# worldbench/lidarcrafter

Hardware: AMD Instinct MI355X
Metric: denoising-steps/sec, nuScenes 32×1024 range image, 1/2/4/8 GPU (higher is better)
Workload: dtype f16x2-split MFMA, fp32 accumulate (fp32-class accuracy)

## Files before the change

lidarcrafter_amd/csrc/conv_f16x2_s2.hip:

```cpp
#include "conv_f16x2_common.h"

using namespace lcconv;

namespace {

#include "conv_f16x2_ps.h"

typedef _Float16 half8_s2 __attribute__((ext_vector_type(8)));

__global__ __launch_bounds__(256) void fir_down2_prefilter_split_kernel(
    const float* __restrict__ x, long long x_bs, half8_s2* __restrict__ ysp, int C8, int H, int W, int nstrip, int strip_len,
    lc_conv_range* range) {
    const int Wh = W >> 1;
    const int i = blockIdx.x * 256 + threadIdx.x;
    const int c8 = blockIdx.y;
    const int b = blockIdx.z / nstrip, strip = blockIdx.z - b * nstrip;
    const float xs = range->x_scale, seen = range->amax_scaled;
    float am = 0.f;
    if (i < Wh) {
        const long long HW = (long long)H * W;
        const float* xb = x + b * x_bs + (long long)c8 * 8 * HW;
        const int R = H + 3;
        half8_s2* yh = ysp + ((long long)b * 2 * C8 + c8) * R * W;
        half8_s2* yl = yh + (long long)C8 * R * W;
        const int cm1 = (2 * i - 1 + W) % W, cp2 = (2 * i + 2) % W;
        constexpr float f0 = 0.125f, f1 = 0.375f, f2 = 0.375f, f3 = 0.125f;
        struct Raw { float a[8]; float2 m[8], c[8]; };
        auto load_raw = [&](int r, Raw& w) {
            const int rc = r < 0 ? 0 : (r >= H ? H - 1 : r);
            const float* p = xb + (long long)rc * W;
#pragma unroll
            for (int k = 0; k < 8; ++k) {
                const float* q = p + (long long)k * HW;
                w.a[k] = q[cm1];
                w.m[k] = *reinterpret_cast<const float2*>(q + 2 * i);
                w.c[k] = *reinterpret_cast<const float2*>(q + cp2);
            }
        };
        auto xw_row = [&](int r, const Raw& w, float (&e)[8], float (&o)[8]) {
            const float in = (r >= 0 && r < H) ? 1.0f : 0.0f;
#pragma unroll
            for (int k = 0; k < 8; ++k) {
                e[k] = in * fmaf(f3, w.c[k].x, fmaf(f2, w.m[k].y, fmaf(f1, w.m[k].x, f0 * w.a[k])));
                o[k] = in * fmaf(f3, w.c[k].y, fmaf(f2, w.c[k].x, fmaf(f1, w.m[k].y, f0 * w.m[k].x)));
            }
        };
        auto put = [&](int row, const float (&e)[8], const float (&o)[8]) {
            half8 h, l;
            split8(e, xs, h, l, am);
            yh[(long long)row * W + Wh + i] = h;
            yl[(long long)row * W + Wh + i] = l;
            const int jo = i + 1 == Wh ? 0 : i + 1;
            split8(o, xs, h, l, am);
            yh[(long long)row * W + jo] = h;
            yl[(long long)row * W + jo] = l;
        };
        const int m0 = -1 + strip * strip_len;
        const int m1 = (m0 + strip_len < H) ? m0 + strip_len : H;
        float we[4][8], wo[4][8];
        Raw raw;
        load_raw(m0 - 1, raw); xw_row(m0 - 1, raw, we[0], wo[0]);
        load_raw(m0, raw); xw_row(m0, raw, we[1], wo[1]);
        load_raw(m0 + 1, raw); xw_row(m0 + 1, raw, we[2], wo[2]);
        load_raw(m0 + 2, raw);
        for (int m = m0; m < m1; ++m) {
            xw_row(m + 2, raw, we[3], wo[3]);
            if (m + 1 < m1) load_raw(m + 3, raw);
            float fe[8], fo[8];
#pragma unroll
            for (int k = 0; k < 8; ++k) {
                fe[k] = fmaf(f3, we[3][k], fmaf(f2, we[2][k], fmaf(f1, we[1][k], f0 * we[0][k])));
                fo[k] = fmaf(f3, wo[3][k], fmaf(f2, wo[2][k], fmaf(f1, wo[1][k], f0 * wo[0][k])));
            }
            put(m + 1, fe, fo);
            if (m == 1) {
#pragma unroll
                for (int k = 0; k < 8; ++k) {
                    fe[k] = fmaf(f3, we[3][k], fmaf(f2, we[2][k], f1 * we[1][k]));
                    fo[k] = fmaf(f3, wo[3][k], fmaf(f2, wo[2][k], f1 * wo[1][k]));
                }
                put(H + 1, fe, fo);
            }
            if (m == H - 3) {
#pragma unroll
                for (int k = 0; k < 8; ++k) {
                    fe[k] = fmaf(f2, we[2][k], fmaf(f1, we[1][k], f0 * we[0][k]));
                    fo[k] = fmaf(f2, wo[2][k], fmaf(f1, wo[1][k], f0 * wo[0][k]));
                }
                put(H + 2, fe, fo);
            }
#pragma unroll
            for (int k = 0; k < 8; ++k) {
                we[0][k] = we[1][k]; we[1][k] = we[2][k]; we[2][k] = we[3][k];
                wo[0][k] = wo[1][k]; wo[1][k] = wo[2][k]; wo[2][k] = wo[3][k];
            }
        }
    }
    publish_amax(range, am, seen);
}

using S2Cfg_ = HCfg<2, 2, 1, 1, 1, 64, 3>;

template <int TPB, bool EMIT_STATS>
__global__ __launch_bounds__(256, 1) void conv_s2_shared_w_kernel(ConvArgsH a) {
    using C = S2Cfg_;
    constexpr int CB = 2, NTAP = 9, BN = 64, TW = 64;
    constexpr int XW = 2 * TW + 1, XR = 3, XU = CB * XR * XW, WU = NTAP * CB * BN;
    constexpr int NWV = 4;
    constexpr int NXI = (XU + 63) / 64, NWI = (WU + 63) / 64;
    constexpr int XS = NXI * 64, WS = NWI * 64;
    constexpr int KX = (2 * NXI + NWV - 1) / NWV, KW = (2 * NWI + NWV - 1) / NWV;
    constexpr unsigned OOB = 0x80000000u;
    __shared__ half8 xlds[2][2 * XS];
    __shared__ half8 wlds[2][2 * WS];
    __shared__ half8 dummy[64];
    const int tid = threadIdx.x, lane = tid & 63;
    const int wave = __builtin_amdgcn_readfirstlane(tid >> 6);
    const int wco = wave >> 1, wpx = wave & 1;
    const int kh = lane >> 5, l31 = lane & 31;

    int bx = blockIdx.x;
    if (a.xcd) bx = (bx & 7) * (gridDim.x >> 3) + (bx >> 3);
    const int gh_ = a.tiles_h / TPB;
    const int tw_i = bx % a.tiles_w; bx /= a.tiles_w;
    const int h0 = (bx % gh_) * TPB; bx /= gh_;
    const int b = bx;
    const int w0 = tw_i * TW;
    const int co0 = blockIdx.y * BN;
    const int H = a.H, W = a.W, HW = H * W;
// ... 176 lines not shown
            for (int m = 0; m < 4; ++m) {
                const int co_oct = co0 + wco * 32 + 8 * m;
                const float sh = half_sum_to_lane31_63(st_s[m]), qh = half_sum_to_lane31_63(st_q[m]);
                const float sf = dpp_add<0x143, 0xC>(sh), qf = dpp_add<0x143, 0xC>(qh);
                const int ent = quads ? (co_oct >> 2) + (lane >> 5) : (co_oct >> 3);
                const unsigned eo = (mine && co_oct < a.Co && gh < H)
                                        ? ((unsigned)ent * (unsigned)a.oslots + (unsigned)slot) * 16u + 4u * (lane & 3)
                                        : OOB;
                store_entry_4lanes(rs_o, st_p[m], nv, quads ? sh : sf, quads ? qh : qf, eo);
            }
        }
    }
}

using S2Cfg = HCfg<2, 2, 1, 1, 1, 64, 3>;

}

extern "C" int64_t lc_conv2d_ring_s2_stats_slots(int Ho, int Wo) {
    if (Ho <= 0 || Wo <= 0 || Wo % S2Cfg::TW_) return 0;
    return (int64_t)Ho * (Wo / S2Cfg::TW_) * S2Cfg::WPX_;
}

extern "C" int64_t lc_fir_down2_split_units(int B, int C, int H, int W) {
    if (B <= 0 || C <= 0 || C % 8 || H <= 0 || W <= 0) return 0;
    return (int64_t)B * 2 * (C / 8) * (H + 3) * W;
}

extern "C" int lc_fir_down2_prefilter_split(const float* x, int64_t x_bs, void* y_split, int B, int C, int H, int W,
                                            lc_conv_range* range, lc_stream_t s) {
    if (!x || !y_split || !range || B <= 0 || C <= 0 || H <= 0 || W <= 0) return LC_EINVAL;
    if (C % 16 || H % 2 || H < 4 || W % 128) return LC_EUNSUP;
    if ((reinterpret_cast<uintptr_t>(x) & 7) || (x_bs & 1)) return LC_EUNSUP;
    int strip_len = 8;
    static const int strip_env = [] { const char* e = getenv("LC_PF_STRIP"); return e ? atoi(e) : 0; }();
    if (strip_env > 0) strip_len = strip_env;
    const int nstrip = (H + 1 + strip_len - 1) / strip_len;
    if ((long long)B * nstrip > 65535) return LC_EUNSUP;
    dim3 grid((W / 2 + 255) / 256, C / 8, B * nstrip);
    hipLaunchKernelGGL(fir_down2_prefilter_split_kernel, grid, dim3(256), 0, lc_s(s), x, (long long)x_bs,
                       reinterpret_cast<half8_s2*>(y_split), C / 8, H, W, nstrip, strip_len, range);
    return lc_launch_status();
}

extern "C" int lc_conv2d_ring_s2_f16x2_ps_fwd(const void* x_split, const void* wp_hi, const void* wp_lo, const float* bias,
                                              float* y, int64_t y_bs, int B, int Ci, int Co, int Ho, int Wo, float out_scale,
                                              float* gn_ostats_out, int gn_ostats_unit, const float* wmeta,
                                              lc_conv_range* range, lc_stream_t s) {
    using C = S2Cfg;
    if (!x_split || !wp_hi || !wp_lo || !y || !wmeta || !range || B <= 0 || Ci <= 0 || Co <= 0 || Ho <= 0 || Wo <= 0)
        return LC_EINVAL;
    if (Ci % 16 || Ho < 2 || Wo % C::TW_) return LC_EUNSUP;
    const long long plane_units = (long long)(Ci / 8) * (2 * Ho + 3) * (2 * Wo);
    if (2 * plane_units * 16 >= (1ll << 31) || (long long)Co * Ho * Wo * 4 >= (1ll << 31)) return LC_EUNSUP;
    ConvArgsH a;
    a.x = nullptr; a.wh = (const half8*)wp_hi; a.wl = (const half8*)wp_lo; a.bias = bias; a.res = nullptr;
    a.y = y; a.x_bs = 0; a.res_bs = 0; a.y_bs = y_bs;
    a.range = range; a.wmeta = wmeta;
    a.B = B; a.Ci = Ci; a.Co = Co; a.H = Ho; a.W = Wo;
    a.Cib = Ci / 8; a.Cop = (Co + 63) / 64 * 64;
    if (a.wl != a.wh + (long long)9 * a.Cib * a.Cop) return LC_EINVAL;
    a.xsp = (const half8*)x_split; a.xsp_c8 = Ci / 8; a.xsp_bs = 2 * plane_units;
    a.part = nullptr; a.ksplit = 0;
    a.out_scale = out_scale;
    a.gn = nullptr; a.Cgn = 0; a.gn_silu = 0;
    a.gs = lc_gn_stats_input{nullptr, 0, 0, 0.f, nullptr, nullptr, nullptr, nullptr, 0, nullptr, nullptr};
    a.seg[0] = a.seg[1] = ConvArgsH::OctSeg{nullptr, 0, 0, 3};
    a.ostats = nullptr; a.oslots = 0; a.ounit = 8;
    if (gn_ostats_out) {
        if (Co % 8 || (gn_ostats_unit != 8 && gn_ostats_unit != 4)) return LC_EUNSUP;
        a.oslots = (int)lc_conv2d_ring_s2_stats_slots(Ho, Wo);
        a.ostats = reinterpret_cast<f32x4*>(gn_ostats_out);
// ... 30 lines not shown
```

lidarcrafter_amd/csrc/resample.hip:

```cpp
#include "common.h"

namespace {

#pragma clang fp contract(off)

struct PairArgs {
    const f32x4* coef; int Cpad; float* y2; long long y2_bs;
};
__device__ __forceinline__ float pair_act(float v, const f32x4& r) { return lc_silu((v - r.x) * r.y + r.z); }

template <bool PAIR>
__global__ __launch_bounds__(256) void down2_kernel(const float* __restrict__ x, long long x_bs,
                                                   float* __restrict__ y, long long y_bs, int C,
                                                   int H, int W, PairArgs pa) {
    const int Ho = H / 2, Wo = W / 2;
    const long long total = (long long)C * Ho * Wo;
    const int b = blockIdx.y;
    const float* xb = x + b * x_bs;
    float* yb = y + b * y_bs;
    float* y2b = PAIR ? pa.y2 + b * pa.y2_bs : nullptr;
    for (long long e = blockIdx.x * 256ll + threadIdx.x; e < total; e += (long long)gridDim.x * 256) {
        const int j = e % Wo;
        const long long r = e / Wo;
        const int i = r % Ho;
        const int c = r / Ho;
        const float* xc = xb + (long long)c * H * W;
        int cols[4];
#pragma unroll
        for (int q = 0; q < 4; ++q) {
            int w = 2 * j + q - 1;
            cols[q] = w < 0 ? w + W : (w >= W ? w - W : w);
        }
        float acc = 0.f, acc2 = 0.f;
// ... 114 lines not shown
                const float xm = row[jm], x0 = row[j], xp = row[jp];
                ev[d] = 0.25f * xm + 0.75f * x0;
                od[d] = 0.75f * x0 + 0.25f * xp;
                if (PAIR) {
                    const float am = pair_act(xm, cr), a0 = pair_act(x0, cr), ap = pair_act(xp, cr);
                    ev2[d] = 0.25f * am + 0.75f * a0;
                    od2[d] = 0.75f * a0 + 0.25f * ap;
                }
            } else {
                ev[d] = 0.f; od[d] = 0.f;
            }
        }
        float* yc = yb + (long long)c * 4 * H * W + (long long)(2 * i) * W2 + 2 * j;
        float2 top, bot;
        top.x = 0.25f * ev[0] + 0.75f * ev[1];
        top.y = 0.25f * od[0] + 0.75f * od[1];
        bot.x = 0.75f * ev[1] + 0.25f * ev[2];
        bot.y = 0.75f * od[1] + 0.25f * od[2];
        lc_st2(yc, top);
        lc_st2(yc + W2, bot);
        if (PAIR) {
            float* yc2 = y2b + (long long)c * 4 * H * W + (long long)(2 * i) * W2 + 2 * j;
            float2 t2, b2;
            t2.x = 0.25f * ev2[0] + 0.75f * ev2[1];
            t2.y = 0.25f * od2[0] + 0.75f * od2[1];
            b2.x = 0.75f * ev2[1] + 0.25f * ev2[2];
            b2.y = 0.75f * od2[1] + 0.25f * od2[2];
            lc_st2(yc2, t2);
            lc_st2(yc2 + W2, b2);
        }
    }
}

}

extern "C" int64_t lc_resample2x_stats_slots(int H, int W, int dir) {
    if (dir >= 0 || H <= 0 || W <= 0 || (H & 1) || W % 256) return 0;
    return (int64_t)(H / 2) * (W / 256);
}

static int resample2x(const float* x, int64_t x_bs, float* y, int64_t y_bs, int B, int C, int H, int W, int dir,
                      float* ostats, lc_stream_t s, const float* coef = nullptr, int Cpad = 0, float* y2 = nullptr,
                      int64_t y2_bs = 0);

extern "C" int lc_resample2x_pair_fwd(const float* x, int64_t x_bs, const float* coeffs, int Cpad, float* y, int64_t y_bs,
                                      float* y_act, int64_t ya_bs, int B, int C, int H, int W, int dir, lc_stream_t s) {
    if (!coeffs || !y_act || Cpad < C) return LC_EINVAL;
    return resample2x(x, x_bs, y, y_bs, B, C, H, W, dir, nullptr, s, coeffs, Cpad, y_act, ya_bs);
}

extern "C" int lc_resample2x_fwd(const float* x, int64_t x_bs, float* y, int64_t y_bs, int B, int C,
                                 int H, int W, int dir, lc_stream_t s) {
    return resample2x(x, x_bs, y, y_bs, B, C, H, W, dir, nullptr, s);
}

extern "C" int lc_resample2x_stats_fwd(const float* x, int64_t x_bs, float* y, int64_t y_bs, int B, int C,
                                       int H, int W, int dir, float* ostats, lc_stream_t s) {
    if (!ostats) return LC_EINVAL;
    return resample2x(x, x_bs, y, y_bs, B, C, H, W, dir, ostats, s);
}

static int resample2x(const float* x, int64_t x_bs, float* y, int64_t y_bs, int B, int C, int H, int W, int dir,
                      float* ostats, lc_stream_t s, const float* coef, int Cpad, float* y2, int64_t y2_bs) {
    if (!x || !y || B <= 0 || C <= 0 || H <= 0 || W <= 0) return LC_EINVAL;
    if (ostats && dir >= 0) return LC_EUNSUP;
    const bool pair = y2 != nullptr;
    const PairArgs pa{reinterpret_cast<const f32x4*>(coef), Cpad, y2, (long long)y2_bs};
    if (dir < 0) {
        if ((H & 1) || (W & 1)) return LC_EUNSUP;
        const long long total = (long long)C * (H / 2) * (W / 2);
        const bool vec = W % 256 == 0 && (x_bs & 3) == 0 && (y_bs & 1) == 0 &&
                         (reinterpret_cast<uintptr_t>(x) & 15) == 0 &&
                         (reinterpret_cast<uintptr_t>(y) & 7) == 0 &&
                         (!pair || ((y2_bs & 1) == 0 && (reinterpret_cast<uintptr_t>(y2) & 7) == 0));
        if (vec) {
            const long long items = (long long)C * (H / 2) * (W / 256);
            int blocks = (int)((items + 3) / 4 > 16384 ? 16384 : (items + 3) / 4);
            if (pair)
                hipLaunchKernelGGL(down2_vec_kernel<true>, dim3(blocks, B), dim3(256), 0, lc_s(s), x,
                                   (long long)x_bs, y, (long long)y_bs, C, H, W, (f32x4*)nullptr, pa);
            else
                hipLaunchKernelGGL(down2_vec_kernel<false>, dim3(blocks, B), dim3(256), 0, lc_s(s), x,
                                   (long long)x_bs, y, (long long)y_bs, C, H, W, reinterpret_cast<f32x4*>(ostats), pa);
            return lc_launch_status();
        }
        if (ostats) return LC_EUNSUP;
        int blocks = (int)((total + 255) / 256 > 8192 ? 8192 : (total + 255) / 256);
        if (pair)
            hipLaunchKernelGGL(down2_kernel<true>, dim3(blocks, B), dim3(256), 0, lc_s(s), x, (long long)x_bs, y,
                               (long long)y_bs, C, H, W, pa);
        else
            hipLaunchKernelGGL(down2_kernel<false>, dim3(blocks, B), dim3(256), 0, lc_s(s), x, (long long)x_bs, y,
                               (long long)y_bs, C, H, W, pa);
    } else {
        if (((y_bs | (int64_t)(2 * W)) & 1) || (reinterpret_cast<uintptr_t>(y) & 7)) return LC_EUNSUP;
        if (pair && ((y2_bs & 1) || (reinterpret_cast<uintptr_t>(y2) & 7))) return LC_EUNSUP;
        const long long total = (long long)C * H * W;
        int blocks = (int)((total + 255) / 256 > 8192 ? 8192 : (total + 255) / 256);
        if (pair)
            hipLaunchKernelGGL(up2_kernel<true>, dim3(blocks, B), dim3(256), 0, lc_s(s), x, (long long)x_bs, y,
                               (long long)y_bs, C, H, W, pa);
        else
            hipLaunchKernelGGL(up2_kernel<false>, dim3(blocks, B), dim3(256), 0, lc_s(s), x, (long long)x_bs, y,
                               (long long)y_bs, C, H, W, pa);
    }
    return lc_launch_status();
}

LC_TOUCH_TU(resample, down2_kernel<false>)
```

lidarcrafter_amd/csrc/upfold.hip:

```cpp
#include "common.h"

namespace {

typedef _Float16 half8_t __attribute__((ext_vector_type(8)));
typedef _Float16 half2_t __attribute__((ext_vector_type(2)));
typedef float float2_t __attribute__((ext_vector_type(2)));

__global__ __launch_bounds__(256) void split_plain_kernel(const float* __restrict__ x, long long x_bs,
                                                         half8_t* __restrict__ ysp, long long ysp_bs, int C,
                                                         long long HW, lc_conv_range* range) {
    const int oct = blockIdx.y, b = blockIdx.z;
    const float* xp = x + b * x_bs + (long long)oct * 8 * HW;
    const float xs = range->x_scale;
    const float seen = range->amax_scaled;
    half8_t* yh = ysp + b * ysp_bs + (long long)oct * HW;
    half8_t* yl = yh + (long long)(C >> 3) * HW;
    float am = 0.0f;
    for (long long tb = blockIdx.x * 1024ll; tb < HW; tb += (long long)gridDim.x * 1024) {
        const long long p = tb + threadIdx.x;
        f32x4 pix[8];
#pragma unroll
        for (int i = 0; i < 4; ++i) {
            const long long pi = p + 256 * i < HW - 1 ? p + 256 * i : HW - 1;
#pragma unroll
            for (int k = 0; k < 8; ++k) pix[k][i] = xp[(long long)k * HW + pi];
        }
#pragma unroll
        for (int i = 0; i < 4; ++i) {
            half8_t h8, l8;
#pragma unroll
            for (int k = 0; k < 8; k += 2) {
                const float s0 = pix[k][i] * xs, s1 = pix[k + 1][i] * xs;
                am = fmaxf(am, fmaxf(fabsf(s0), fabsf(s1)));
// ... 16 lines not shown
__device__ __forceinline__ float hz0(float p0m, float p0, float p1m, float p1, float p2, float p2p) {
    float s = 0.75f * p0m;
    s = fmaf(0.25f, p0, s);
    s = fmaf(0.25f, p1m, s);
    s = fmaf(0.75f, p1, s);
    s = fmaf(0.75f, p2, s);
    return fmaf(0.25f, p2p, s);
}
__device__ __forceinline__ float hz1(float p0m, float p0, float p1, float p1p, float p2, float p2p) {
    float s = 0.25f * p0m;
    s = fmaf(0.75f, p0, s);
    s = fmaf(0.75f, p1, s);
    s = fmaf(0.25f, p1p, s);
    s = fmaf(0.25f, p2, s);
    return fmaf(0.75f, p2p, s);
}

struct XupArgs { const float* x; long long x_bs; float* y2; long long y2_bs; };
#pragma clang fp contract(off)
__device__ __forceinline__ void xup_row(float xm, float xa, float xb, float xp, float (&o)[4]) {
    o[0] = 0.25f * xm + 0.75f * xa;
    o[1] = 0.75f * xa + 0.25f * xb;
    o[2] = 0.25f * xa + 0.75f * xb;
    o[3] = 0.75f * xb + 0.25f * xp;
}
__device__ __forceinline__ float xup_top(float m, float c) { return 0.25f * m + 0.75f * c; }
__device__ __forceinline__ float xup_bot(float c, float p) { return 0.75f * c + 0.25f * p; }
#pragma clang fp contract(fast)

template <bool STATS, bool XUP>
__global__ __launch_bounds__(256) void up2_combine9_kernel(const float* __restrict__ p9, long long p_bs,
                                                          const float* __restrict__ bias, float* __restrict__ y,
                                                          long long y_bs, int Co, int H, int W,
                                                          f32x4* __restrict__ ostats, XupArgs xa) {
    const int segs = W >> 7;
    const int item = blockIdx.x * 4 + __builtin_amdgcn_readfirstlane((int)(threadIdx.x >> 6));
    if (item >= Co * segs) return;
    const int lane = threadIdx.x & 63, b = blockIdx.y;
    const int co = item / segs, sg = item - co * segs;
    const int j0 = sg * 128 + 2 * lane;
    const int jm = j0 == 0 ? W - 1 : j0 - 1, jp = j0 + 2 == W ? 0 : j0 + 2;
    const long long HW = (long long)H * W, ts = (long long)Co * HW;
    const float* pb = p9 + b * p_bs + (long long)co * HW;
    const float bs = bias ? bias[co] : 0.0f;
    float* yc = y + b * y_bs + (long long)co * 4 * HW;
    const __amdgpu_buffer_rsrc_t rs_y = lc_wt_buf(yc);
    const unsigned col_off = (unsigned)(2 * j0) * 4u, row_bytes = (unsigned)(2 * W) * 4u;

    float L[9], A[9], Bv[9], R[9];
    float xl = 0.f, xc0 = 0.f, xc1 = 0.f, xr = 0.f;
    const float* xb_ = XUP ? xa.x + b * xa.x_bs + (long long)co * HW : nullptr;
    auto load_row = [&](int i) {
        const float* row = pb + (long long)i * W;
#pragma unroll
        for (int t = 0; t < 9; ++t) {
            const float* q = row + t * ts;
            const float2 v = *reinterpret_cast<const float2*>(q + j0);
            L[t] = q[jm]; A[t] = v.x; Bv[t] = v.y; R[t] = q[jp];
        }
        if (XUP) {
            const float* q = xb_ + (long long)i * W;
            const float2 v = *reinterpret_cast<const float2*>(q + j0);
            xl = q[jm]; xc0 = v.x; xc1 = v.y; xr = q[jp];
        }
    };
    float Xm[4] = {0.f, 0.f, 0.f, 0.f}, X0[4] = {0.f, 0.f, 0.f, 0.f}, Xp[4] = {0.f, 0.f, 0.f, 0.f};
    auto xrow = [&](float (&o)[4], bool inside) {
        xup_row(xl, xc0, xc1, xr, o);
        if (!inside) { o[0] = 0.f; o[1] = 0.f; o[2] = 0.f; o[3] = 0.f; }
    };
    float* y2c = XUP ? xa.y2 + b * xa.y2_bs + (long long)co * 4 * HW : nullptr;
    const __amdgpu_buffer_rsrc_t rs_y2 = lc_wt_buf(y2c);
    auto horiz = [&](float (&Hh)[3][4], float f) {
#pragma unroll
        for (int ky = 0; ky < 3; ++ky) {
            const int t0 = 3 * ky, t1 = t0 + 1, t2 = t0 + 2;
            Hh[ky][0] = f * hz0(L[t0], A[t0], L[t1], A[t1], A[t2], Bv[t2]);
            Hh[ky][1] = f * hz1(L[t0], A[t0], A[t1], Bv[t1], A[t2], Bv[t2]);
            Hh[ky][2] = f * hz0(A[t0], Bv[t0], A[t1], Bv[t1], Bv[t2], R[t2]);
            Hh[ky][3] = f * hz1(A[t0], Bv[t0], Bv[t1], R[t1], Bv[t2], R[t2]);
        }
    };
    float Hm[3][4], H0[3][4], Hp[3][4];
#pragma unroll
    for (int ky = 0; ky < 3; ++ky)
#pragma unroll
        for (int c = 0; c < 4; ++c) Hm[ky][c] = 0.0f;
    load_row(0);
    horiz(H0, 1.0f);
    if (XUP) xrow(X0, true);
    load_row(H > 1 ? 1 : 0);
    horiz(Hp, H > 1 ? 1.0f : 0.0f);
    if (XUP) xrow(Xp, H > 1);
    for (int i = 0; i < H; ++i) {
        load_row(i + 2 < H ? i + 2 : H - 1);
        const float ft = i > 0 ? 1.0f : 0.0f, fb = i + 1 < H ? 1.0f : 0.0f;
        f32x4 top, bot;
#pragma unroll
        for (int c = 0; c < 4; ++c) {
            float t = ft * fmaf(0.25f, H0[0][c], 0.75f * Hm[0][c]);
            t = fmaf(0.25f, Hm[1][c], t);
            t = fmaf(0.75f, H0[1][c], t);
            t = fmaf(0.75f, H0[2][c], t);
            t = fmaf(0.25f, Hp[2][c], t);
            top[c] = t + bs;
            float u = fb * fmaf(0.75f, Hp[2][c], 0.25f * H0[2][c]);
            u = fmaf(0.25f, Hm[0][c], u);
            u = fmaf(0.75f, H0[0][c], u);
            u = fmaf(0.75f, H0[1][c], u);
            u = fmaf(0.25f, Hp[1][c], u);
            bot[c] = u + bs;
        }
        const unsigned off = (unsigned)(2 * i) * row_bytes + col_off;
        lc_st4(rs_y, off, top);
        lc_st4(rs_y, off + row_bytes, bot);
        if (XUP) {
            f32x4 xt, xb2;
#pragma unroll
            for (int c = 0; c < 4; ++c) { xt[c] = xup_top(Xm[c], X0[c]); xb2[c] = xup_bot(X0[c], Xp[c]); }
            lc_st4(rs_y2, off, xt);
            lc_st4(rs_y2, off + row_bytes, xb2);
        }
        if (STATS) {
            const float piv = __builtin_amdgcn_readfirstlane(top[0]);
            float s_ = 0.0f, q_ = 0.0f;
#pragma unroll
            for (int c = 0; c < 4; ++c) {
                const float d0 = top[c] - piv, d1 = bot[c] - piv;
                s_ += d0 + d1;
                q_ = fmaf(d0, d0, q_);
                q_ = fmaf(d1, d1, q_);
            }
#pragma unroll
            for (int sh = 32; sh > 0; sh >>= 1) { s_ += __shfl_xor(s_, sh, 64); q_ += __shfl_xor(q_, sh, 64); }
            if (lane == 0)
                ostats[((long long)b * Co + co) * ((long long)H * segs) + ((long long)i * segs + sg)] = f32x4{piv, 512.0f, s_, q_};
        }
        float Hn[3][4];
        horiz(Hn, i + 2 < H ? 1.0f : 0.0f);
        if (XUP) {
            float Xn[4];
            xrow(Xn, i + 2 < H);
#pragma unroll
            for (int c = 0; c < 4; ++c) { Xm[c] = X0[c]; X0[c] = Xp[c]; Xp[c] = Xn[c]; }
        }
#pragma unroll
        for (int ky = 0; ky < 3; ++ky)
#pragma unroll
            for (int c = 0; c < 4; ++c) { Hm[ky][c] = H0[ky][c]; H0[ky][c] = Hp[ky][c]; Hp[ky][c] = Hn[ky][c]; }
    }
}

}

extern "C" int lc_split_act_fwd(const float* x, int64_t x_bs, void* y_split, int B, int C, int H, int W,
                                lc_conv_range* range, lc_stream_t s) {
    if (!x || !y_split || !range || B <= 0 || C <= 0 || H <= 0 || W <= 0) return LC_EINVAL;
    const long long HW = (long long)H * W;
    if (C % 16 || HW % 4 || (x_bs & 3) || (reinterpret_cast<uintptr_t>(x) & 15)) return LC_EUNSUP;
    if (2ll * (C / 8) * HW * 16 >= (1ll << 31)) return LC_EUNSUP;
    long long gx = (HW + 1023) / 1024;
    while (gx > 1 && gx * (C / 8) * B > 8192) gx = (gx + 1) / 2;
    hipLaunchKernelGGL(split_plain_kernel, dim3((unsigned)gx, C / 8, B), dim3(256), 0, lc_s(s), x, (long long)x_bs,
                       reinterpret_cast<half8_t*>(y_split), (long long)2 * (C / 8) * HW, C, HW, range);
    return lc_launch_status();
}

extern "C" int64_t lc_up2_combine9_stats_slots(int H, int W) {
    if (H <= 0 || W <= 0 || W % 128) return 0;
    return (int64_t)H * (W / 128);
}

static int up2_combine9(const float* p9, int64_t p_bs, const float* bias, float* y, int64_t y_bs, int B, int Co, int H, int W,
                        float* ostats, const float* x, int64_t x_bs, float* y2, int64_t y2_bs, lc_stream_t s) {
    if (!p9 || !y || B <= 0 || Co <= 0 || H <= 0 || W <= 0) return LC_EINVAL;
    if (W % 128 || (p_bs & 1) || (y_bs & 3) || (reinterpret_cast<uintptr_t>(p9) & 7) ||
        (reinterpret_cast<uintptr_t>(y) & 15))
        return LC_EUNSUP;
    if (x && ((x_bs & 1) || (y2_bs & 3) || (reinterpret_cast<uintptr_t>(x) & 7) || (reinterpret_cast<uintptr_t>(y2) & 15)))
        return LC_EUNSUP;
    if (16ll * H * W >= (1ll << 32)) return LC_EUNSUP;
    const long long items = (long long)Co * (W / 128);
    const dim3 grid((unsigned)((items + 3) / 4), B);
    const XupArgs xa{x, (long long)x_bs, y2, (long long)y2_bs};
    f32x4* os = reinterpret_cast<f32x4*>(ostats);
#define LC_UPC(ST, XU) hipLaunchKernelGGL((up2_combine9_kernel<ST, XU>), grid, dim3(256), 0, lc_s(s), p9, (long long)p_bs, \
                                          bias, y, (long long)y_bs, Co, H, W, os, xa)
    if (ostats) { if (x) LC_UPC(true, true); else LC_UPC(true, false); }
    else { if (x) LC_UPC(false, true); else LC_UPC(false, false); }
#undef LC_UPC
    return lc_launch_status();
}

extern "C" int lc_up2_combine9_fwd(const float* p9, int64_t p_bs, const float* bias, float* y, int64_t y_bs, int B,
                                   int Co, int H, int W, float* ostats, lc_stream_t s) {
    return up2_combine9(p9, p_bs, bias, y, y_bs, B, Co, H, W, ostats, nullptr, 0, nullptr, 0, s);
}

extern "C" int lc_up2_combine9_xup_fwd(const float* p9, int64_t p_bs, const float* bias, float* y, int64_t y_bs,
                                       const float* x, int64_t x_bs, float* y2, int64_t y2_bs, int B, int Co, int H, int W,
                                       float* ostats, lc_stream_t s) {
    if (!x || !y2) return LC_EINVAL;
    return up2_combine9(p9, p_bs, bias, y, y_bs, B, Co, H, W, ostats, x, x_bs, y2, y2_bs, s);
}

LC_TOUCH_TU(upfold, up2_combine9_kernel<true, false>)
```

Baseline: 274.4.

## Use DPP lane shifts for halo columns and pipeline row loads in resample kernels

Replaces the scattered per-thread halo column loads in the down2 prefilter and up2 combine kernels with one wave-cooperative halo load, distributed via DPP lane shifts and readlane. Rows are double-buffered so the next rows load while the current one computes. The combine kernel gains a row split (hsplit) for more parallelism, and a new row-streaming up2 kernel is added. This cuts redundant global loads and raises occupancy on small feature maps, at the cost of more registers, per-call getenv, and extra recomputed halo rows for split strips.

```diff
diff --git a/devtools/resample_ab.py b/devtools/resample_ab.py
--- /dev/null
+++ b/devtools/resample_ab.py
@@ -0,0 +1,142 @@
+import ctypes as ct
+import os
+import sys
+
+sys.path.insert(0, os.path.dirname(os.path.dirname(os.path.abspath(__file__))))
+import torch
+
+from lidarcrafter_amd._lib import SIGNATURES
+from lidarcrafter_amd.testing import seeded_randn
+from tests.test_resample_streams import PF_SHAPES, UP2_SHAPES, UP9_SHAPES
+
+NAMES = ("lc_fir_down2_prefilter_split", "lc_fir_down2_split_units", "lc_up2_combine9_fwd", "lc_up2_combine9_xup_fwd",
+         "lc_up2_combine9_stats_slots", "lc_resample2x_fwd", "lc_resample2x_pair_fwd")
+ENVS = ("LC_PF_STRIP", "LC_UP9_HSPLIT", "LC_UP2_HSPLIT", "LC_UP2_ROWS")
+for k in ENVS:
+    os.environ.pop(k, None)
+dev = torch.device("cuda:0")
+sweep = "--sweep" in sys.argv
+libs = []
+for path in [a for a in sys.argv[1:] if not a.startswith("--")]:
+    h = ct.CDLL(os.path.abspath(path))
+    for n in NAMES:
+        f = getattr(h, n)
+        f.restype, f.argtypes = SIGNATURES[n]
+    libs.append((os.path.basename(path), h))
+st = torch.cuda.current_stream().cuda_stream
+
+
+def pf(h, a):
+    x = a["x"]
+    B, C, H, W = x.shape
+    buf = torch.full((int(h.lc_fir_down2_split_units(B, C, H, W)), 8), -7.0, device=dev, dtype=torch.float16)
+    rng = torch.tensor([16.0, 1 / 16.0, 0.0, 0.0], device=dev)
+    go = lambda: h.lc_fir_down2_prefilter_split(x.data_ptr(), x.stride(0), buf.data_ptr(), B, C, H, W, rng.data_ptr(), st)
+    return go, (buf, rng)
+
+
+def up9(h, a):
+    p9, bias, x, stats = a["p9"], a["bias"], a["x"], a["stats"]
+    B, C9, H, W = p9.shape
+    Co = C9 // 9
+    y = torch.full((B, Co, 2 * H, 2 * W), -7.0, device=dev)
+    ent = torch.full((B, Co, int(h.lc_up2_combine9_stats_slots(H, W)), 4), -7.0, device=dev)
+    y2 = torch.full((B, Co, 2 * H, 2 * W) if x is not None else (1,), -7.0, device=dev)
+    sp = ent.data_ptr() if stats else None
+    if x is None:
+        go = lambda: h.lc_up2_combine9_fwd(p9.data_ptr(), p9.stride(0), bias.data_ptr(), y.data_ptr(), y.stride(0), B, Co, H, W, sp, st)
+    else:
+        go = lambda: h.lc_up2_combine9_xup_fwd(p9.data_ptr(), p9.stride(0), bias.data_ptr(), y.data_ptr(), y.stride(0), x.data_ptr(),
+                                               x.stride(0), y2.data_ptr(), y2.stride(0), B, Co, H, W, sp, st)
+    return go, (y, ent, y2)
+
+
+def up2(h, a):
+    x, coef = a["x"], a["coef"]
+    B, C, H, W = x.shape
+    y = torch.full((B, C, 2 * H, 2 * W), -7.0, device=dev)
+    ya = torch.full((B, C, 2 * H, 2 * W) if coef is not None else (1,), -7.0, device=dev)
+    if coef is None:
+        go = lambda: h.lc_resample2x_fwd(x.data_ptr(), x.stride(0), y.data_ptr(), y.stride(0), B, C, H, W, 1, st)
+    else:
+        go = lambda: h.lc_resample2x_pair_fwd(x.data_ptr(), x.stride(0), coef.data_ptr(), coef.shape[1], y.data_ptr(), y.stride(0),
+                                              ya.data_ptr(), ya.stride(0), B, C, H, W, 1, st)
+    return go, (y, ya)
+
+
+def clock(go):
+    best = 1e9
+    for _ in range(5):
+        e0, e1 = torch.cuda.Event(enable_timing=True), torch.cuda.Event(enable_timing=True)
+        e0.record()
+        for _ in range(50):
+            go()
+        e1.record()
+        torch.cuda.synchronize()
+        best = min(best, e0.elapsed_time(e1) / 50 * 1e3)
+    return best
+
+
+def rnd(*shape, seed):
+    return (seeded_randn(*shape, seed=seed) * 1.3 - 0.2).to(dev)
+
+
+def coefs(B, C):
+    c = torch.zeros(B, C + 1, 4)
+    c[..., 0], c[..., 1], c[..., 2] = 0.1 * seeded_randn(B, C + 1, seed=1), 1 + 0.2 * seeded_randn(B, C + 1, seed=2), 0.3 * seeded_randn(B, C + 1, seed=3)
+    return c.to(dev)
+
+
+cases = []
+for B, C, H, W in ((8, 64, 32, 1024), (8, 128, 16, 512), (8, 256, 8, 256)):
+    cases.append((f"C2 pre-filter {B}x{C}x{H}x{W}", pf, dict(x=rnd(B, C, H, W, seed=5)), True, {"LC_PF_STRIP": (8, 6, 5, 4, 3, 2, 1)}))
+for B, Co, H, W in ((8, 128, 8, 256), (8, 256, 4, 128)):
+    cases.append((f"C2 combine {B}x{Co}x{H}x{W}", up9, dict(p9=rnd(B, 9 * Co, H, W, seed=6), bias=rnd(Co, seed=7), x=None, stats=True),
+                  True, {"LC_UP9_HSPLIT": (1, 2, 4)}))
+cases.append(("C2 up2 8x64x16x512", up2, dict(x=rnd(8, 64, 16, 512, seed=8), coef=None), True,
+              {"LC_UP2_HSPLIT": (1, 2, 4, 8), "LC_UP2_ROWS": (0,)}))
+for B, C, H, W in PF_SHAPES:
+    cases.append((f"test pre-filter {B}x{C}x{H}x{W}", pf, dict(x=rnd(B, C, H, W, seed=3 * H + W)), False, None))
+for W, H in UP9_SHAPES:
+    for stats in (True, False):
+        for xup in (False, True):
+            cases.append((f"test combine {W}x{H} stats {int(stats)} xup {int(xup)}", up9,
+                          dict(p9=rnd(2, 27, H, W, seed=400 + H + W), bias=rnd(3, seed=5), x=rnd(2, 3, H, W, seed=31 + H) if xup else None,
+                               stats=stats), False, None))
+for H, W in UP2_SHAPES:
+    for pair in (False, True):
+        cases.append((f"test up2 {H}x{W} pair {int(pair)}", up2, dict(x=rnd(2, 3, H, W, seed=12 + H + W), coef=coefs(2, 3) if pair else None),
+                      False, None))
+
+ok = True
+for tag, fn, a, timed, envs in cases:
+    ref, line = None, []
+    for name, h in libs:
+        go, outs = fn(h, a)
+        rc = go()
+        assert rc == 0, (tag, name, rc)
+        torch.cuda.synchronize()
+        if ref is None:
+            ref, same = outs, "ref"
+        else:
+            bad = [i for i, (p, q) in enumerate(zip(outs, ref)) if not torch.equal(p, q)]
+            ok &= not bad
+            same = "equal" if not bad else f"DIFFERENT (tensor {bad[0]})"
+        line.append(f"{name} {same}" + (f" {clock(go):6.2f} us" if timed else ""))
+    print(f"{tag:36s} | " + " | ".join(line), flush=True)
+    if sweep and envs:
+        for k, vals in envs.items():
+            for v in vals:
+                os.environ[k] = str(v)
+                line = []
+                for name, h in libs[1:]:
+                    go, outs = fn(h, a)
+                    assert go() == 0
+                    torch.cuda.synchronize()
+                    eq = all(torch.equal(p, q) for p, q in zip(outs, ref))
+                    ok &= eq
+                    line.append(f"{name} {'equal' if eq else 'DIFFERENT'} {clock(go):6.2f} us")
+                print(f"    {k}={v:<3d} | " + " | ".join(line), flush=True)
+            del os.environ[k]
+print("BIT-IDENTICAL" if ok else "OUTPUTS DIFFER")
+sys.exit(0 if ok else 1)
diff --git a/devtools/resample_report.py b/devtools/resample_report.py
--- /dev/null
+++ b/devtools/resample_report.py
@@ -0,0 +1,50 @@
+import collections
+import csv
+import sys
+
+PAT = ("fir_down2_prefilter_split_kernel", "up2_combine9_kernel", "up2_kernel", "up2_rows_kernel")
+rows = list(csv.DictReader(open(sys.argv[1])))
+label = sys.argv[2] if len(sys.argv) > 2 else sys.argv[1]
+pmc = "Counter_Name" in rows[0]
+key_t = "Start_Timestamp" if not pmc else "Dispatch_Id"
+disp = collections.OrderedDict()
+for r in sorted(rows, key=lambda r: int(r[key_t])):
+    d = int(r["Dispatch_Id"])
+    if "Grid_Size_X" in r:
+        grid = tuple(int(r[f"Grid_Size_{a}"]) // int(r[f"Workgroup_Size_{a}"]) for a in "XYZ")
+    else:
+        grid = (int(r["Grid_Size"]) // int(r["Workgroup_Size"]),)
+    if d not in disp:
+        disp[d] = [r["Kernel_Name"], grid, {} if pmc else (int(r["End_Timestamp"]) - int(r["Start_Timestamp"])) / 1e3]
+    if pmc:
+        disp[d][2][r["Counter_Name"]] = float(r["Counter_Value"])
+
+steps, cur = [], []
+for name, grid, val in disp.values():
+    if "pstep" in name:
+        steps.append(cur)
+        cur = []
+    else:
+        for p in PAT:
+            if p in name:
+                cur.append((p[:24], grid, val))
+                break
+steps = [s for s in steps[2:] if len(s) == len(steps[-1])]
+print(f"# {label}: {len(steps)} steps of {len(steps[-1]) if steps else 0} resampling launches")
+if not steps:
+    sys.exit(0)
+total = 0.0
+for i in range(len(steps[0])):
+    name, grid, _ = steps[0][i]
+    if not pmc:
+        v = [s[i][2] for s in steps]
+        total += sum(v) / len(v)
+        print(f"{i:3d} {name:24s} grid {str(grid):16s} mean {sum(v) / len(v):6.2f} us  min {min(v):6.2f} us")
+    else:
+        out = []
+        for c in sorted(steps[0][i][2]):
+            v = [s[i][2][c] for s in steps if c in s[i][2]]
+            out.append(f"{c} {sum(v) / len(v):.0f}")
+        print(f"{i:3d} {name:24s} grid {str(grid):16s} " + "  ".join(out))
+if not pmc:
+    print(f"# all {len(steps[0])} launches: {total:.1f} us per step")
diff --git a/lidarcrafter_amd/csrc/conv_f16x2_s2.hip b/lidarcrafter_amd/csrc/conv_f16x2_s2.hip
--- a/lidarcrafter_amd/csrc/conv_f16x2_s2.hip
+++ b/lidarcrafter_amd/csrc/conv_f16x2_s2.hip
@@ -1,4 +1,5 @@
 #include "conv_f16x2_common.h"
+#include "lane_shift.h"
 
 using namespace lcconv;
 
@@ -11,38 +12,41 @@
 __global__ __launch_bounds__(256) void fir_down2_prefilter_split_kernel(
     const float* __restrict__ x, long long x_bs, half8_s2* __restrict__ ysp, int C8, int H, int W, int nstrip, int strip_len,
     lc_conv_range* range) {
-    const int Wh = W >> 1;
-    const int i = blockIdx.x * 256 + threadIdx.x;
-    const int c8 = blockIdx.y;
-    const int b = blockIdx.z / nstrip, strip = blockIdx.z - b * nstrip;
+    const int Wh = W >> 1, segs = Wh >> 6;
+    const int lane = threadIdx.x & 63;
+    const int item = blockIdx.x * 4 + __builtin_amdgcn_readfirstlane((int)(threadIdx.x >> 6));
+    const int c8 = blockIdx.y, b = blockIdx.z;
     const float xs = range->x_scale, seen = range->amax_scaled;
     float am = 0.f;
-    if (i < Wh) {
+    if (item < segs * nstrip) {
+        const int sg = item / nstrip, strip = item - sg * nstrip;
+        const int i = sg * 64 + lane;
         const long long HW = (long long)H * W;
         const float* xb = x + b * x_bs + (long long)c8 * 8 * HW;
         const int R = H + 3;
         half8_s2* yh = ysp + ((long long)b * 2 * C8 + c8) * R * W;
         half8_s2* yl = yh + (long long)C8 * R * W;
-        const int cm1 = (2 * i - 1 + W) % W, cp2 = (2 * i + 2) % W;
+        const int hk = lane < 24 ? lane / 3 : 0, hq = lane < 24 ? lane - 3 * hk : 0;
+        const int hleft = sg == 0 ? W - 1 : 128 * sg - 1, hright = sg + 1 == segs ? 0 : 128 * (sg + 1);
+        const long long hoff = (long long)hk * HW + (hq == 0 ? hleft : hright + hq - 1);
         constexpr float f0 = 0.125f, f1 = 0.375f, f2 = 0.375f, f3 = 0.125f;
-        struct Raw { float a[8]; float2 m[8], c[8]; };
+        struct Raw { float2 m[8]; float h; };
         auto load_raw = [&](int r, Raw& w) {
             const int rc = r < 0 ? 0 : (r >= H ? H - 1 : r);
             const float* p = xb + (long long)rc * W;
 #pragma unroll
-            for (int k = 0; k < 8; ++k) {
-                const float* q = p + (long long)k * HW;
-                w.a[k] = q[cm1];
-                w.m[k] = *reinterpret_cast<const float2*>(q + 2 * i);
-                w.c[k] = *reinterpret_cast<const float2*>(q + cp2);
-            }
+            for (int k = 0; k < 8; ++k) w.m[k] = *reinterpret_cast<const float2*>(p + (long long)k * HW + 2 * i);
+            w.h = p[hoff];
         };
         auto xw_row = [&](int r, const Raw& w, float (&e)[8], float (&o)[8]) {
             const float in = (r >= 0 && r < H) ? 1.0f : 0.0f;
 #pragma unroll
             for (int k = 0; k < 8; ++k) {
-                e[k] = in * fmaf(f3, w.c[k].x, fmaf(f2, w.m[k].y, fmaf(f1, w.m[k].x, f0 * w.a[k])));
-                o[k] = in * fmaf(f3, w.c[k].y, fmaf(f2, w.c[k].x, fmaf(f1, w.m[k].y, f0 * w.m[k].x)));
+                const float a = lc_from_left(w.m[k].y, lc_lane_bcast(w.h, 3 * k));
+                const float cx = lc_from_right(w.m[k].x, lc_lane_bcast(w.h, 3 * k + 1));
+                const float cy = lc_from_right(w.m[k].y, lc_lane_bcast(w.h, 3 * k + 2));
+                e[k] = in * fmaf(f3, cx, fmaf(f2, w.m[k].y, fmaf(f1, w.m[k].x, f0 * a)));
+                o[k] = in * fmaf(f3, cy, fmaf(f2, cx, fmaf(f1, w.m[k].y, f0 * w.m[k].x)));
             }
         };
         auto put = [&](int row, const float (&e)[8], const float (&o)[8]) {
@@ -58,14 +62,18 @@
         const int m0 = -1 + strip * strip_len;
         const int m1 = (m0 + strip_len < H) ? m0 + strip_len : H;
         float we[4][8], wo[4][8];
-        Raw raw;
-        load_raw(m0 - 1, raw); xw_row(m0 - 1, raw, we[0], wo[0]);
-        load_raw(m0, raw); xw_row(m0, raw, we[1], wo[1]);
-        load_raw(m0 + 1, raw); xw_row(m0 + 1, raw, we[2], wo[2]);
-        load_raw(m0 + 2, raw);
-        for (int m = m0; m < m1; ++m) {
-            xw_row(m + 2, raw, we[3], wo[3]);
-            if (m + 1 < m1) load_raw(m + 3, raw);
+        Raw ra, rb;
+        {
+            Raw p0, p1, p2;
+            load_raw(m0 - 1, p0); load_raw(m0, p1); load_raw(m0 + 1, p2);
+            load_raw(m0 + 2, ra); load_raw(m0 + 3, rb);
+            xw_row(m0 - 1, p0, we[0], wo[0]);
+            xw_row(m0, p1, we[1], wo[1]);
+            xw_row(m0 + 1, p2, we[2], wo[2]);
+            xw_row(m0 + 2, ra, we[3], wo[3]);
+        }
+        auto step = [&](int m, Raw& mine, const Raw& other, bool more, bool next) {
+            if (more) load_raw(m + 4, mine);
             float fe[8], fo[8];
 #pragma unroll
             for (int k = 0; k < 8; ++k) {
@@ -94,7 +102,16 @@
                 we[0][k] = we[1][k]; we[1][k] = we[2][k]; we[2][k] = we[3][k];
                 wo[0][k] = wo[1][k]; wo[1][k] = wo[2][k]; wo[2][k] = wo[3][k];
             }
-        }
+            if (next) xw_row(m + 3, other, we[3], wo[3]);
+        };
+        int m = m0;
+        for (; m + 3 < m1; m += 2) {
+            step(m, ra, rb, true, true);
+            step(m + 1, rb, ra, true, true);
+        }
+        step(m, ra, rb, m + 2 < m1, m + 1 < m1);
+        if (m + 1 < m1) step(m + 1, rb, ra, false, m + 2 < m1);
+        if (m + 2 < m1) step(m + 2, ra, rb, false, false);
     }
     publish_amax(range, am, seen);
 }
@@ -337,12 +354,14 @@
     if (!x || !y_split || !range || B <= 0 || C <= 0 || H <= 0 || W <= 0) return LC_EINVAL;
     if (C % 16 || H % 2 || H < 4 || W % 128) return LC_EUNSUP;
     if ((reinterpret_cast<uintptr_t>(x) & 7) || (x_bs & 1)) return LC_EUNSUP;
-    int strip_len = 8;
-    static const int strip_env = [] { const char* e = getenv("LC_PF_STRIP"); return e ? atoi(e) : 0; }();
+    const int segs = W / 128;
+    int strip_len = H <= 8 ? 3 : 8;
+    const char* strip_e = getenv("LC_PF_STRIP");
+    const int strip_env = strip_e ? atoi(strip_e) : 0;
     if (strip_env > 0) strip_len = strip_env;
     const int nstrip = (H + 1 + strip_len - 1) / strip_len;
-    if ((long long)B * nstrip > 65535) return LC_EUNSUP;
-    dim3 grid((W / 2 + 255) / 256, C / 8, B * nstrip);
+    if (B > 65535 || C / 8 > 65535) return LC_EUNSUP;
+    dim3 grid((segs * nstrip + 3) / 4, C / 8, B);
     hipLaunchKernelGGL(fir_down2_prefilter_split_kernel, grid, dim3(256), 0, lc_s(s), x, (long long)x_bs,
                        reinterpret_cast<half8_s2*>(y_split), C / 8, H, W, nstrip, strip_len, range);
     return lc_launch_status();
diff --git a/lidarcrafter_amd/csrc/lane_shift.h b/lidarcrafter_amd/csrc/lane_shift.h
--- /dev/null
+++ b/lidarcrafter_amd/csrc/lane_shift.h
@@ -0,0 +1,30 @@
+#pragma once
+#include "common.h"
+
+#ifndef LC_LANE_SHIFT_BPERMUTE
+#define LC_LANE_SHIFT_BPERMUTE 0
+#endif
+
+__device__ __forceinline__ float lc_from_left(float v, float edge) {
+#if LC_LANE_SHIFT_BPERMUTE
+    const float s = __shfl_up(v, 1, 64);
+    return (threadIdx.x & 63) == 0 ? edge : s;
+#else
+    return __builtin_bit_cast(float, __builtin_amdgcn_update_dpp(__builtin_bit_cast(int, edge), __builtin_bit_cast(int, v),
+                                                                 0x138, 0xF, 0xF, false));
+#endif
+}
+
+__device__ __forceinline__ float lc_from_right(float v, float edge) {
+#if LC_LANE_SHIFT_BPERMUTE
+    const float s = __shfl_down(v, 1, 64);
+    return (threadIdx.x & 63) == 63 ? edge : s;
+#else
+    return __builtin_bit_cast(float, __builtin_amdgcn_update_dpp(__builtin_bit_cast(int, edge), __builtin_bit_cast(int, v),
+                                                                 0x130, 0xF, 0xF, false));
+#endif
+}
+
+__device__ __forceinline__ float lc_lane_bcast(float v, int l) {
+    return __builtin_bit_cast(float, __builtin_amdgcn_readlane(__builtin_bit_cast(int, v), l));
+}
diff --git a/lidarcrafter_amd/csrc/resample.hip b/lidarcrafter_amd/csrc/resample.hip
--- a/lidarcrafter_amd/csrc/resample.hip
+++ b/lidarcrafter_amd/csrc/resample.hip
@@ -1,4 +1,6 @@
 #include "common.h"
+#include "lane_shift.h"
+#include <cstdlib>
 
 namespace {
 
@@ -179,6 +181,99 @@
     }
 }
 
+template <bool PAIR>
+__global__ __launch_bounds__(256) void up2_rows_kernel(const float* __restrict__ x, long long x_bs,
+                                                      float* __restrict__ y, long long y_bs, int C,
+                                                      int H, int W, PairArgs pa, int hsplit) {
+    const int segs = W >> 7;
+    const int item = blockIdx.x * 4 + __builtin_amdgcn_readfirstlane((int)(threadIdx.x >> 6));
+    if (item >= C * segs * hsplit) return;
+    const int lane = threadIdx.x & 63, b = blockIdx.y;
+    const int cs = item / hsplit, part = item - cs * hsplit;
+    const int c = cs / segs, sg = cs - c * segs;
+    const int rows = (H + hsplit - 1) / hsplit;
+    const int r0 = part * rows, r1 = r0 + rows < H ? r0 + rows : H;
+    if (r0 >= r1) return;
+    const int j0 = sg * 128 + 2 * lane;
+    const long long HW = (long long)H * W;
+    const float* xc = x + b * x_bs + (long long)c * HW;
+    const __amdgpu_buffer_rsrc_t rs_y = lc_wt_buf(y + b * y_bs + (long long)c * 4 * HW);
+    const __amdgpu_buffer_rsrc_t rs_y2 = lc_wt_buf(PAIR ? pa.y2 + b * pa.y2_bs + (long long)c * 4 * HW : nullptr);
+    const unsigned col_off = (unsigned)(2 * j0) * 4u, row_bytes = (unsigned)(2 * W) * 4u;
+    const int hleft = sg == 0 ? W - 1 : sg * 128 - 1, hright = sg + 1 == segs ? 0 : (sg + 1) * 128;
+    const float* hp = xc + (lane == 1 ? hright : hleft);
+    f32x4 cr = {0.f, 0.f, 0.f, 0.f};
+    if (PAIR) cr = pa.coef[(long long)b * pa.Cpad + c];
+
+    struct Raw { float2 v; float h; };
+    auto load_row = [&](int i, Raw& w) {
+        w.v = *reinterpret_cast<const float2*>(xc + (long long)i * W + j0);
+        w.h = hp[(long long)i * W];
+    };
+    auto hrow = [&](const Raw& w, bool inside, float (&o)[4], float (&o2)[4]) {
+        const float xl = lc_from_left(w.v.y, lc_lane_bcast(w.h, 0)), xr = lc_from_right(w.v.x, lc_lane_bcast(w.h, 1));
+        o[0] = 0.25f * xl + 0.75f * w.v.x;
+        o[1] = 0.75f * w.v.x + 0.25f * w.v.y;
+        o[2] = 0.25f * w.v.x + 0.75f * w.v.y;
+        o[3] = 0.75f * w.v.y + 0.25f * xr;
+        if (PAIR) {
+            const float aa = pair_act(w.v.x, cr), ab = pair_act(w.v.y, cr), ah = pair_act(w.h, cr);
+            const float al = lc_from_left(ab, lc_lane_bcast(ah, 0)), ar = lc_from_right(aa, lc_lane_bcast(ah, 1));
+            o2[0] = 0.25f * al + 0.75f * aa;
+            o2[1] = 0.75f * aa + 0.25f * ab;
+            o2[2] = 0.25f * aa + 0.75f * ab;
+            o2[3] = 0.75f * ab + 0.25f * ar;
+        }
+        if (!inside) {
+#pragma unroll
+            for (int q = 0; q < 4; ++q) { o[q] = 0.f; o2[q] = 0.f; }
+        }
+    };
+    auto clampr = [&](int i) { return i < H ? i : H - 1; };
+    float Xm[4] = {0.f, 0.f, 0.f, 0.f}, X0[4], Xp[4], Ym[4] = {0.f, 0.f, 0.f, 0.f}, Y0[4], Yp[4];
+    Raw ra, rb;
+    {
+        Raw p0, p1, p2;
+        if (r0 > 0) load_row(r0 - 1, p0);
+        load_row(r0, p1); load_row(clampr(r0 + 1), p2);
+        load_row(clampr(r0 + 2), ra); load_row(clampr(r0 + 3), rb);
+        if (r0 > 0) hrow(p0, true, Xm, Ym);
+        hrow(p1, true, X0, Y0);
+        hrow(p2, r0 + 1 < H, Xp, Yp);
+    }
+    auto step = [&](int i, Raw& mine, bool more) {
+        f32x4 top, bot;
+#pragma unroll
+        for (int q = 0; q < 4; ++q) { top[q] = 0.25f * Xm[q] + 0.75f * X0[q]; bot[q] = 0.75f * X0[q] + 0.25f * Xp[q]; }
+        const unsigned off = (unsigned)(2 * i) * row_bytes + col_off;
+        lc_st4(rs_y, off, top);
+        lc_st4(rs_y, off + row_bytes, bot);
+        if (PAIR) {
+#pragma unroll
+            for (int q = 0; q < 4; ++q) { top[q] = 0.25f * Ym[q] + 0.75f * Y0[q]; bot[q] = 0.75f * Y0[q] + 0.25f * Yp[q]; }
+            lc_st4(rs_y2, off, top);
+            lc_st4(rs_y2, off + row_bytes, bot);
+        }
+        float Xn[4], Yn[4];
+        hrow(mine, i + 2 < H, Xn, Yn);
+        if (more) load_row(clampr(i + 4), mine);
+#pragma unroll
+        for (int q = 0; q < 4; ++q) {
+            Xm[q] = X0[q]; X0[q] = Xp[q]; Xp[q] = Xn[q];
+            if (PAIR) { Ym[q] = Y0[q]; Y0[q] = Yp[q]; Yp[q] = Yn[q]; }
+        }
+    };
+    int i = r0;
+    for (; i + 4 < r1; i += 2) {
+        step(i, ra, true);
+        step(i + 1, rb, true);
+    }
+    step(i, ra, i + 3 < r1);
+    if (i + 1 < r1) step(i + 1, rb, false);
+    if (i + 2 < r1) step(i + 2, ra, false);
+    if (i + 3 < r1) step(i + 3, rb, false);
+}
+
 }
 
 extern "C" int64_t lc_resample2x_stats_slots(int H, int W, int dir) {
@@ -242,6 +337,27 @@
     } else {
         if (((y_bs | (int64_t)(2 * W)) & 1) || (reinterpret_cast<uintptr_t>(y) & 7)) return LC_EUNSUP;
         if (pair && ((y2_bs & 1) || (reinterpret_cast<uintptr_t>(y2) & 7))) return LC_EUNSUP;
+        const char* form_env = getenv("LC_UP2_ROWS");
+        const bool rows_form = W % 128 == 0 && (x_bs & 1) == 0 && (y_bs & 3) == 0 && (reinterpret_cast<uintptr_t>(x) & 7) == 0 &&
+                               (reinterpret_cast<uintptr_t>(y) & 15) == 0 && 16ll * H * W < (1ll << 32) &&
+                               (!pair || ((y2_bs & 3) == 0 && (reinterpret_cast<uintptr_t>(y2) & 15) == 0)) &&
+                               !(form_env && atoi(form_env) == 0);
+        if (rows_form) {
+            int hsplit = 1;
+            while ((H + hsplit - 1) / hsplit > 4 && (long long)B * C * (W / 128) * hsplit < 2048) hsplit *= 2;
+            const char* hs_env = getenv("LC_UP2_HSPLIT");
+            if (hs_env && atoi(hs_env) > 0) hsplit = atoi(hs_env) < H ? atoi(hs_env) : H;
+            const long long items = (long long)C * (W / 128) * hsplit;
+            if ((items + 3) / 4 > 0x7FFFFFFFll) return LC_EUNSUP;
+            const dim3 grid((unsigned)((items + 3) / 4), B);
+            if (pair)
+                hipLaunchKernelGGL(up2_rows_kernel<true>, grid, dim3(256), 0, lc_s(s), x, (long long)x_bs, y, (long long)y_bs, C,
+                                   H, W, pa, hsplit);
+            else
+                hipLaunchKernelGGL(up2_rows_kernel<false>, grid, dim3(256), 0, lc_s(s), x, (long long)x_bs, y, (long long)y_bs, C,
+                                   H, W, pa, hsplit);
+            return lc_launch_status();
+        }
         const long long total = (long long)C * H * W;
         int blocks = (int)((total + 255) / 256 > 8192 ? 8192 : (total + 255) / 256);
         if (pair)
diff --git a/lidarcrafter_amd/csrc/upfold.hip b/lidarcrafter_amd/csrc/upfold.hip
--- a/lidarcrafter_amd/csrc/upfold.hip
+++ b/lidarcrafter_amd/csrc/upfold.hip
@@ -1,4 +1,6 @@
 #include "common.h"
+#include "lane_shift.h"
+#include <cstdlib>
 
 namespace {
 
@@ -81,36 +83,49 @@
 __global__ __launch_bounds__(256) void up2_combine9_kernel(const float* __restrict__ p9, long long p_bs,
                                                           const float* __restrict__ bias, float* __restrict__ y,
                                                           long long y_bs, int Co, int H, int W,
-                                                          f32x4* __restrict__ ostats, XupArgs xa) {
+                                                          f32x4* __restrict__ ostats, XupArgs xa, int hsplit) {
     const int segs = W >> 7;
     const int item = blockIdx.x * 4 + __builtin_amdgcn_readfirstlane((int)(threadIdx.x >> 6));
-    if (item >= Co * segs) return;
+    if (item >= Co * segs * hsplit) return;
     const int lane = threadIdx.x & 63, b = blockIdx.y;
-    const int co = item / segs, sg = item - co * segs;
+    const int cs = item / hsplit, part = item - cs * hsplit;
+    const int co = cs / segs, sg = cs - co * segs;
+    const int rows = (H + hsplit - 1) / hsplit;
+    const int r0 = part * rows, r1 = r0 + rows < H ? r0 + rows : H;
+    if (r0 >= r1) return;
     const int j0 = sg * 128 + 2 * lane;
-    const int jm = j0 == 0 ? W - 1 : j0 - 1, jp = j0 + 2 == W ? 0 : j0 + 2;
     const long long HW = (long long)H * W, ts = (long long)Co * HW;
     const float* pb = p9 + b * p_bs + (long long)co * HW;
     const float bs = bias ? bias[co] : 0.0f;
     float* yc = y + b * y_bs + (long long)co * 4 * HW;
     const __amdgpu_buffer_rsrc_t rs_y = lc_wt_buf(yc);
     const unsigned col_off = (unsigned)(2 * j0) * 4u, row_bytes = (unsigned)(2 * W) * 4u;
-
+    const float* xb_ = XUP ? xa.x + b * xa.x_bs + (long long)co * HW : nullptr;
+    const int hleft = sg == 0 ? W - 1 : sg * 128 - 1, hright = sg + 1 == segs ? 0 : (sg + 1) * 128;
+    const int hl = lane < (XUP ? 20 : 18) ? lane : 0;
+    const float* hp = (XUP && hl >= 18 ? xb_ : pb + (hl >> 1) * ts) + ((hl & 1) ? hright : hleft);
+
+    struct Raw { float2 v[9]; float2 xv; float h; };
+    auto load_row = [&](int i, Raw& w) {
+        const float* row = pb + (long long)i * W + j0;
+#pragma unroll
+        for (int t = 0; t < 9; ++t) w.v[t] = *reinterpret_cast<const float2*>(row + t * ts);
+        if (XUP) w.xv = *reinterpret_cast<const float2*>(xb_ + (long long)i * W + j0);
+        w.h = hp[(long long)i * W];
+    };
     float L[9], A[9], Bv[9], R[9];
     float xl = 0.f, xc0 = 0.f, xc1 = 0.f, xr = 0.f;
-    const float* xb_ = XUP ? xa.x + b * xa.x_bs + (long long)co * HW : nullptr;
-    auto load_row = [&](int i) {
-        const float* row = pb + (long long)i * W;
+    auto unpack = [&](const Raw& w) {
 #pragma unroll
         for (int t = 0; t < 9; ++t) {
-            const float* q = row + t * ts;
-            const float2 v = *reinterpret_cast<const float2*>(q + j0);
-            L[t] = q[jm]; A[t] = v.x; Bv[t] = v.y; R[t] = q[jp];
+            L[t] = lc_from_left(w.v[t].y, lc_lane_bcast(w.h, 2 * t));
+            A[t] = w.v[t].x; Bv[t] = w.v[t].y;
+            R[t] = lc_from_right(w.v[t].x, lc_lane_bcast(w.h, 2 * t + 1));
         }
         if (XUP) {
-            const float* q = xb_ + (long long)i * W;
-            const float2 v = *reinterpret_cast<const float2*>(q + j0);
-            xl = q[jm]; xc0 = v.x; xc1 = v.y; xr = q[jp];
+            xl = lc_from_left(w.xv.y, lc_lane_bcast(w.h, 18));
+            xc0 = w.xv.x; xc1 = w.xv.y;
+            xr = lc_from_right(w.xv.x, lc_lane_bcast(w.h, 19));
         }
     };
     float Xm[4] = {0.f, 0.f, 0.f, 0.f}, X0[4] = {0.f, 0.f, 0.f, 0.f}, Xp[4] = {0.f, 0.f, 0.f, 0.f};
@@ -130,19 +145,31 @@
             Hh[ky][3] = f * hz1(A[t0], Bv[t0], Bv[t1], R[t1], Bv[t2], R[t2]);
         }
     };
+    auto clampr = [&](int i) { return i < H ? i : H - 1; };
     float Hm[3][4], H0[3][4], Hp[3][4];
-#pragma unroll
-    for (int ky = 0; ky < 3; ++ky)
-#pragma unroll
-        for (int c = 0; c < 4; ++c) Hm[ky][c] = 0.0f;
-    load_row(0);
-    horiz(H0, 1.0f);
-    if (XUP) xrow(X0, true);
-    load_row(H > 1 ? 1 : 0);
-    horiz(Hp, H > 1 ? 1.0f : 0.0f);
-    if (XUP) xrow(Xp, H > 1);
-    for (int i = 0; i < H; ++i) {
-        load_row(i + 2 < H ? i + 2 : H - 1);
+    Raw ra, rb;
+    {
+        Raw p0, p1, p2;
+        if (r0 > 0) load_row(r0 - 1, p0);
+        load_row(r0, p1); load_row(clampr(r0 + 1), p2);
+        load_row(clampr(r0 + 2), ra); load_row(clampr(r0 + 3), rb);
+#pragma unroll
+        for (int ky = 0; ky < 3; ++ky)
+#pragma unroll
+            for (int c = 0; c < 4; ++c) Hm[ky][c] = 0.0f;
+        if (r0 > 0) {
+            unpack(p0);
+            horiz(Hm, 1.0f);
+            if (XUP) xrow(Xm, true);
+        }
+        unpack(p1);
+        horiz(H0, 1.0f);
+        if (XUP) xrow(X0, true);
+        unpack(p2);
+        horiz(Hp, r0 + 1 < H ? 1.0f : 0.0f);
+        if (XUP) xrow(Xp, r0 + 1 < H);
+    }
+    auto step = [&](int i, Raw& mine, bool more) {
         const float ft = i > 0 ? 1.0f : 0.0f, fb = i + 1 < H ? 1.0f : 0.0f;
         f32x4 top, bot;
 #pragma unroll
@@ -186,6 +213,7 @@
                 ostats[((long long)b * Co + co) * ((long long)H * segs) + ((long long)i * segs + sg)] = f32x4{piv, 512.0f, s_, q_};
         }
         float Hn[3][4];
+        unpack(mine);
         horiz(Hn, i + 2 < H ? 1.0f : 0.0f);
         if (XUP) {
             float Xn[4];
@@ -193,11 +221,21 @@
 #pragma unroll
             for (int c = 0; c < 4; ++c) { Xm[c] = X0[c]; X0[c] = Xp[c]; Xp[c] = Xn[c]; }
         }
+        if (more) load_row(clampr(i + 4), mine);
 #pragma unroll
         for (int ky = 0; ky < 3; ++ky)
 #pragma unroll
             for (int c = 0; c < 4; ++c) { Hm[ky][c] = H0[ky][c]; H0[ky][c] = Hp[ky][c]; Hp[ky][c] = Hn[ky][c]; }
+    };
+    int i = r0;
+    for (; i + 4 < r1; i += 2) {
+        step(i, ra, true);
+        step(i + 1, rb, true);
     }
+    step(i, ra, i + 3 < r1);
+    if (i + 1 < r1) step(i + 1, rb, false);
+    if (i + 2 < r1) step(i + 2, ra, false);
+    if (i + 3 < r1) step(i + 3, rb, false);
 }
 
 }
@@ -229,12 +267,18 @@
     if (x && ((x_bs & 1) || (y2_bs & 3) || (reinterpret_cast<uintptr_t>(x) & 7) || (reinterpret_cast<uintptr_t>(y2) & 15)))
         return LC_EUNSUP;
     if (16ll * H * W >= (1ll << 32)) return LC_EUNSUP;
-    const long long items = (long long)Co * (W / 128);
+    int hsplit = 1;
+    while ((H + hsplit - 1) / hsplit > 4 && (long long)B * Co * (W / 128) * hsplit < 4096) hsplit *= 2;
+    const char* hs_env = getenv("LC_UP9_HSPLIT");
+    const int hsplit_env = hs_env ? atoi(hs_env) : 0;
+    if (hsplit_env > 0) hsplit = hsplit_env < H ? hsplit_env : H;
+    const long long items = (long long)Co * (W / 128) * hsplit;
+    if ((items + 3) / 4 > 0x7FFFFFFFll) return LC_EUNSUP;
     const dim3 grid((unsigned)((items + 3) / 4), B);
     const XupArgs xa{x, (long long)x_bs, y2, (long long)y2_bs};
     f32x4* os = reinterpret_cast<f32x4*>(ostats);
 #define LC_UPC(ST, XU) hipLaunchKernelGGL((up2_combine9_kernel<ST, XU>), grid, dim3(256), 0, lc_s(s), p9, (long long)p_bs, \
-                                          bias, y, (long long)y_bs, Co, H, W, os, xa)
+                                          bias, y, (long long)y_bs, Co, H, W, os, xa, hsplit)
     if (ostats) { if (x) LC_UPC(true, true); else LC_UPC(true, false); }
     else { if (x) LC_UPC(false, true); else LC_UPC(false, false); }
 #undef LC_UPC
```

Measured after the change: 276.5 (median of 6 runs). Within noise of the previous version (+0.8%).
